# libjxl/libjxl

Measured on AMD Instinct MI355X. Metric: Mpixels/s decode (VarDCT d1.0, 8K RGB), higher is better.
Workload: dtype f32

## Files before the change

libjxl_amd/csrc/kernels_blocks.hip:

```cpp
#include <stdlib.h>
#include <string.h>

#include <type_traits>

#include <initializer_list>

#include "blocks_common.h"
#include "env_switches.h"

namespace jxlhip {

struct StrategyWord {
  uint32_t v[JXLHIP_NUM_STRATEGIES];
};
__host__ __device__ constexpr StrategyWord MakeStrategyWords() {
  StrategyWord w{};
  for (int s = 0; s < JXLHIP_NUM_STRATEGIES; s++)
    w.v[s] = (uint32_t)kCoveredX[s] | ((uint32_t)kCoveredY[s] << 8) | ((uint32_t)(uint8_t)ClassOfStrategy(s) << 16);
  return w;
}
__constant__ StrategyWord kStrategyWords = MakeStrategyWords();

__global__ __launch_bounds__(1024) void k_prepare(DevFrame f, WorkLists wl, uint32_t gy_lo,
                                                  int with_sigma, float epf_quant_mul,
// ... 254 lines not shown
      for (int iy = 0; iy < 4; iy++)
#pragma unroll
        for (int ix = 0; ix < 8; ix++)
          if (ix | iy) block[iy * 8 + ix] = co[(y + iy * 2) * 8 + ix];
      Idct2dReg<4, 8>(block, out);
#pragma unroll
      for (int iy = 0; iy < 4; iy++)
#pragma unroll
        for (int ix = 0; ix < 8; ix++) px[(y * 4 + iy) * 8 + ix] = out[iy * 8 + ix];
    }
  } else if constexpr (STRATEGY == 13) {
    const float b0 = co[0], b1 = co[8];
    const float dcs[2] = {b0 + b1, b0 - b1};
#pragma unroll
    for (int x = 0; x < 2; x++) {
      float block[32], out[32];
      block[0] = dcs[x];
#pragma unroll
      for (int iy = 0; iy < 4; iy++)
#pragma unroll
        for (int ix = 0; ix < 8; ix++)
          if (ix | iy) block[iy * 8 + ix] = co[(x + iy * 2) * 8 + ix];
      Idct2dReg<8, 4>(block, out);
#pragma unroll
      for (int iy = 0; iy < 8; iy++)
#pragma unroll
        for (int ix = 0; ix < 4; ix++) px[iy * 8 + x * 4 + ix] = out[iy * 4 + ix];
    }
  } else {
    AfvToPixels<STRATEGY - 14>(co, px);
  }
}

struct TabOffsets {
  uint32_t v[27];
};
__host__ __device__ constexpr TabOffsets MakeTabOffsets() {
  TabOffsets t{};
  for (int s = 0; s < 27; s++) t.v[s] = DequantOffset(s);
  return t;
}
static constexpr TabOffsets kSingleTabOffset = MakeTabOffsets();

template <typename CT>
struct Dct8Geom {
  static constexpr int kSteps = sizeof(CT) == 2 ? 4 : 2;
  static constexpr uint32_t kPerWg = 4 * kSteps * 8;
};

template <typename CT>
__device__ __forceinline__ void Dct8Rows(const DevFrame& f, const WorkItem* __restrict__ list, uint32_t n,
                                         uint32_t wg) {
  constexpr int kSteps = Dct8Geom<CT>::kSteps;
  const int lane = threadIdx.x & 63, wave = threadIdx.x >> 6;
  const uint32_t first = (wg * 4 + wave) * (kSteps * 8);
  if (first >= n) return;
  const int j = lane >> 3;
  const bool bit3 = (lane & 8) != 0;
  float tab[3][8];
#pragma unroll
  for (int c = 0; c < 3; c++) {
    const float4 t0 = *(const float4*)(f.dequant + c * 64 + j * 8);
    const float4 t1 = *(const float4*)(f.dequant + c * 64 + j * 8 + 4);
    tab[c][0] = t0.x, tab[c][1] = t0.y, tab[c][2] = t0.z, tab[c][3] = t0.w;
    tab[c][4] = t1.x, tab[c][5] = t1.y, tab[c][6] = t1.z, tab[c][7] = t1.w;
  }
  WorkItem it[kSteps];
  Dct8Row<CT> rows[kSteps][3];
  float dcv[kSteps][3];
  bool valid[kSteps];
#pragma unroll
  for (int s = 0; s < kSteps; s++) {
    const uint32_t b = first + s * 8 + (lane & 7);
    valid[s] = b < n;
    it[s] = list[valid[s] ? b : n - 1];
  }
#pragma unroll
  for (int s = 0; s < kSteps; s++) {
    const size_t elem = (size_t)it[s].off * 64u + (size_t)j * 8u;
    const size_t cell = (size_t)(it[s].pos >> 16) * f.xsb + (it[s].pos & 0xffffu);
#pragma unroll
    for (int c = 0; c < 3; c++) {
      rows[s][c].Load(f.coeffs[c], elem);
      dcv[s][c] = f.dc[c][cell];
    }
  }
#pragma unroll
  for (int s = 0; s < kSteps; s++) {
    const BlockHdr h = MakeHdr(f, it[s]);
    int32_t q[8];
    float vy[8];
    rows[s][1].Unpack(q);
#pragma unroll
    for (int k = 0; k < 8; k++) vy[k] = AdjustQuantBias(q[k], f.biases[1], f.biases[3]) * (tab[1][k] * h.sy);
#pragma unroll
    for (int ci = 0; ci < 3; ci++) {
      const int c = ci == 0 ? 1 : (ci == 1 ? 0 : 2);
      float v[8];
      if (c == 1) {
#pragma unroll
        for (int k = 0; k < 8; k++) v[k] = vy[k];
      } else {
        const float sc = c == 0 ? h.sx : h.sb;
        const float cc = c == 0 ? h.x_cc : h.b_cc;
        rows[s][c].Unpack(q);
#pragma unroll
        for (int k = 0; k < 8; k++) {
          const float d = AdjustQuantBias(q[k], f.biases[c], f.biases[3]) * (tab[c][k] * sc);
          v[k] = __builtin_fmaf(cc, vy[k], d);
        }
      }
      if (j == 0) v[0] = dcv[s][c];
      IdctReg<8>(v);
      Transpose8Lanes(v, bit3);
      IdctReg<8>(v);
      if (valid[s]) {
        float* dst = TilePtr(f, c, it[s].pos >> 16, it[s].pos & 0xffffu) + j * 8;
        *(float4*)dst = make_float4(v[0], v[1], v[2], v[3]);
        *(float4*)(dst + 4) = make_float4(v[4], v[5], v[6], v[7]);
      }
    }
  }
}

template <typename CT>
__device__ __forceinline__ void SpecialTask(const DevFrame& f, int strategy, const WorkItem* __restrict__ list,
                                            uint32_t first, uint32_t n, int c) {
  constexpr int kVec = 64 * (int)sizeof(CT) / 16;
  const int lane = threadIdx.x & 63;
  const uint32_t idx = first + lane;
  const bool valid = idx < n;
  const WorkItem it = list[valid ? idx : n - 1];
  const BlockHdr h = MakeHdr(f, it);
  const float* __restrict__ tab = f.dequant + kSingleTabOffset.v[strategy];
  const float dcv = f.dc[c][(size_t)h.aby * f.xsb + h.abx];
  auto unpack = [&](const uint4 r, int32_t* q) {
    const uint32_t w[4] = {r.x, r.y, r.z, r.w};
    if constexpr (sizeof(CT) == 2) {
#pragma unroll
      for (int k = 0; k < 4; k++) {
        q[2 * k] = (int32_t)(int16_t)(w[k] & 0xffffu);
        q[2 * k + 1] = (int32_t)w[k] >> 16;
      }
    } else {
#pragma unroll
      for (int k = 0; k < 4; k++) q[k] = (int32_t)w[k];
    }
  };
  constexpr int kPer = 16 / (int)sizeof(CT);
  float v[64], px[64];
  {
    const uint4* p = (const uint4*)((const CT*)f.coeffs[1] + h.coef);
    uint4 raw[kVec];
#pragma unroll
    for (int i = 0; i < kVec; i++) raw[i] = p[i];
#pragma unroll
    for (int i = 0; i < kVec; i++) {
      int32_t q[kPer];
      unpack(raw[i], q);
#pragma unroll
      for (int k = 0; k < kPer; k++)
        v[i * kPer + k] = AdjustQuantBias(q[k], f.biases[1], f.biases[3]) * (tab[64 + i * kPer + k] * h.sy);
    }
  }
  if (c != 1) {
    const float sc = c == 0 ? h.sx : h.sb;
    const float cc = c == 0 ? h.x_cc : h.b_cc;
    const float bias = c == 0 ? f.biases[0] : f.biases[2];
    const float* __restrict__ tc = tab + c * 64;
    const uint4* p = (const uint4*)((const CT*)f.coeffs[c] + h.coef);
    uint4 raw[kVec];
#pragma unroll
    for (int i = 0; i < kVec; i++) raw[i] = p[i];
#pragma unroll
    for (int i = 0; i < kVec; i++) {
      int32_t q[kPer];
      unpack(raw[i], q);
#pragma unroll
      for (int k = 0; k < kPer; k++) {
        const float d = AdjustQuantBias(q[k], bias, f.biases[3]) * (tc[i * kPer + k] * sc);
        v[i * kPer + k] = __builtin_fmaf(cc, v[i * kPer + k], d);
      }
    }
  }
  v[0] = dcv;
  switch (strategy) {
    case 1: Transform64<1>(v, px); break;
    case 2: Transform64<2>(v, px); break;
    case 3: Transform64<3>(v, px); break;
    case 12: Transform64<12>(v, px); break;
    case 13: Transform64<13>(v, px); break;
    case 14: Transform64<14>(v, px); break;
    case 15: Transform64<15>(v, px); break;
    case 16: Transform64<16>(v, px); break;
    default: Transform64<17>(v, px); break;
  }
  if (valid) {
    float4* dst = (float4*)TilePtr(f, c, h.aby, h.abx);
#pragma unroll
    for (int i = 0; i < 16; i++) dst[i] = make_float4(px[4 * i], px[4 * i + 1], px[4 * i + 2], px[4 * i + 3]);
  }
}

template <typename CT>
__device__ __forceinline__ uint32_t SpecialWorkgroup(const DevFrame& f, const WorkLists& wl, uint32_t wg) {
  uint32_t cnt[kNumSpecial];
  uint32_t tasks = 0;
#pragma unroll
  for (int i = 0; i < kNumSpecial; i++) {
    cnt[i] = wl.count[(kClsSpecial0 + i) * kCounterPad];
    tasks += 3 * ((cnt[i] + 63) / 64);
  }
  const uint32_t special_wgs = (tasks + 3) / 4;
  if (wg >= special_wgs) return special_wgs;
  const uint32_t task = wg * 4 + (threadIdx.x >> 6);
  if (task >= tasks) return special_wgs;
  uint32_t base = 0;
  int cls = -1;
  uint32_t first = 0, n = 0, chan = 0;
#pragma unroll
  for (int i = 0; i < kNumSpecial; i++) {
    const uint32_t t = 3 * ((cnt[i] + 63) / 64);
    if (cls < 0 && task < base + t) {
      cls = i;
      first = ((task - base) / 3) * 64;
      chan = (task - base) % 3;
      n = cnt[i];
    }
    base += t;
  }
  SpecialTask<CT>(f, (int)kSpecialStrategy[cls], wl.list[kClsSpecial0 + cls], first, n,
                  chan == 0 ? 1 : (chan == 1 ? 0 : 2));
  return special_wgs;
}

template <typename CT>
__global__ __launch_bounds__(256, 3) void k_transform_8(DevFrame f, WorkLists wl) {
  const uint32_t special_wgs = SpecialWorkgroup<CT>(f, wl, blockIdx.x);
  if (blockIdx.x >= special_wgs)
    Dct8Rows<CT>(f, wl.list[kClsDct8], wl.count[kClsDct8 * kCounterPad], blockIdx.x - special_wgs);
}

template <int BIT>
__device__ __forceinline__ void ExchangePair(float& a, float& b, int lane) {
  if constexpr (BIT == 5) {
    SwapHalves32(a, b);
  } else if constexpr (BIT == 4) {
    SwapRows16(a, b);
  } else {
    const bool set = (lane >> BIT) & 1;
    const float send = set ? a : b;
    float recv;
    if constexpr (BIT == 3) {
      recv = __int_as_float(__builtin_amdgcn_update_dpp(0, __float_as_int(send), 0x128, 0xf, 0xf, false));
    } else if constexpr (BIT == 2) {
      const float lo = __int_as_float(__builtin_amdgcn_update_dpp(0, __float_as_int(send), 0x124, 0xf, 0xf, false));
      const float hi = __int_as_float(__builtin_amdgcn_update_dpp(0, __float_as_int(send), 0x12c, 0xf, 0xf, false));
      recv = set ? lo : hi;
    } else {
      static_assert(BIT == 1, "lane bits 1..5");
      recv = __int_as_float(__builtin_amdgcn_update_dpp(0, __float_as_int(send), 0x4e, 0xf, 0xf, false));
    }
    a = set ? recv : a;
    b = set ? b : recv;
  }
}

template <int S>
__device__ __forceinline__ void TransposeTile(float* w, int lane) {
  constexpr int kLog = S == 8 ? 3 : (S == 16 ? 4 : 5);
  constexpr int kLb0 = 6 - kLog;
#pragma unroll
  for (int t = kLog - 1; t >= 0; t--) {
#pragma unroll
    for (int k = 0; k < S; k++) {
      if (k & (1 << t)) continue;
      if (kLb0 + t == 5) ExchangePair<5>(w[k], w[k | (1 << t)], lane);
      else if (kLb0 + t == 4) ExchangePair<4>(w[k], w[k | (1 << t)], lane);
      else if (kLb0 + t == 3) ExchangePair<3>(w[k], w[k | (1 << t)], lane);
      else if (kLb0 + t == 2) ExchangePair<2>(w[k], w[k | (1 << t)], lane);
      else ExchangePair<1>(w[k], w[k | (1 << t)], lane);
    }
  }
}

typedef __attribute__((address_space(3))) float LdsTile;
template <int S>
__device__ __forceinline__ void TransposeTileLds(float* w, int b, int j, LdsTile* wave_lds) {
  LdsTile* tile = wave_lds + b * (S * (S + 1));
  LdsTile* row = tile + j * (S + 1);
#pragma unroll
  for (int a = 0; a < S; a++) row[a] = w[a];
  __builtin_amdgcn_fence(__ATOMIC_RELEASE, "wavefront");
  __builtin_amdgcn_wave_barrier();
  __builtin_amdgcn_fence(__ATOMIC_ACQUIRE, "wavefront");
#pragma unroll
  for (int a = 0; a < S; a++) w[a] = tile[a * (S + 1) + j];
  __builtin_amdgcn_fence(__ATOMIC_RELEASE, "wavefront");
  __builtin_amdgcn_wave_barrier();
}
template <int S>
constexpr int TransposeLdsBytes() { return 4 * (64 / S) * S * (S + 1) * 4; }

template <int R, int C, int STRATEGY, typename CT, bool LDS_T = false>
__device__ __forceinline__ void RowLaneUnit(const DevFrame& f, const WorkItem* __restrict__ list,
                                            uint32_t first, uint32_t n, unsigned char* smem = nullptr) {
  constexpr int S = R < C ? R : C, L = R < C ? C : R;
  constexpr int BPS = 64 / S;
  constexpr int CY = R / 8, CX = C / 8;
  constexpr int kTiles = L / S;
  constexpr int kVec = L * (int)sizeof(CT) / 16;
  const int tid = Tid();
  const int lane = tid & 63, wave = tid >> 6;
  const int j = lane / BPS;
  const uint32_t vb = first + wave * BPS + (lane & (BPS - 1));
  if (first + wave * BPS >= n) return;
  const bool valid = vb < n;
  const WorkItem it = list[valid ? vb : n - 1];
  const BlockHdr h = MakeHdr(f, it);
  uint4 raw_a[kVec], raw_b[kVec];
  auto request = [&](int c, uint4* r) {
    const uint4* p = (const uint4*)((const CT*)f.coeffs[c] + h.coef + (size_t)j * L);
#pragma unroll
    for (int i = 0; i < kVec; i++) r[i] = p[i];
  };
  request(1, raw_a);
  request(0, raw_b);
  constexpr int kLlfLanes = CY < CX ? CY : CX;
  constexpr int kLlfRegs = CY < CX ? CX : CY;
  auto llf_of = [&](int c, float* out) {
    const float* dc = f.dc[c] + (size_t)h.aby * f.xsb + h.abx;
    float dp[CY][CX];
#pragma unroll
    for (int x = 0; x < CX; x++) {
      float v[CY];
#pragma unroll
      for (int y = 0; y < CY; y++) v[y] = dc[(size_t)y * f.xsb + x];
      DctReg<CY>(v);
#pragma unroll
      for (int y = 0; y < CY; y++) dp[y][x] = (1.0f / CY) * v[y];
    }
#pragma unroll
    for (int y = 0; y < CY; y++) {
      float v[CX];
#pragma unroll
      for (int x = 0; x < CX; x++) v[x] = dp[y][x];
      DctReg<CX>(v);
      const float ry = kResampleUpHost[CY + y];
#pragma unroll
      for (int x = 0; x < CX; x++) {
        const float val = (1.0f / CX) * v[x];
        if constexpr (CY < CX) {
          if (j == y) out[x] = val * ry * kResampleUpHost[CX + x];
        } else {
          if (j == x) out[y] = val * kResampleUpHost[CX + x] * ry;
        }
      }
    }
  };
  const float* __restrict__ tab = f.dequant + DequantOffset(STRATEGY) + j * L;
  constexpr int kPer = 16 / (int)sizeof(CT);
  auto unpack_piece = [&](const uint4 r, int32_t* q) {
    if constexpr (sizeof(CT) == 2) {
      const uint32_t w[4] = {r.x, r.y, r.z, r.w};
#pragma unroll
      for (int k = 0; k < 4; k++) {
        q[2 * k] = (int32_t)(int16_t)(w[k] & 0xffffu);
        q[2 * k + 1] = (int32_t)w[k] >> 16;
      }
    } else {
      q[0] = (int32_t)r.x, q[1] = (int32_t)r.y, q[2] = (int32_t)r.z, q[3] = (int32_t)r.w;
    }
  };
  float vy[L];
#pragma unroll
  for (int i = 0; i < kVec; i++) {
    int32_t q[kPer];
    unpack_piece(raw_a[i], q);
#pragma unroll
    for (int k = 0; k < kPer; k++)
      vy[i * kPer + k] = AdjustQuantBias(q[k], f.biases[1], f.biases[3]) * (tab[R * C + i * kPer + k] * h.sy);
    if constexpr (L > 16) __builtin_amdgcn_sched_barrier(0);
  }
  request(2, raw_a);
#pragma unroll
  for (int ci = 0; ci < 3; ci++) {
    const int c = ci == 0 ? 1 : (ci == 1 ? 0 : 2);
    float v[L];
    if (c == 1) {
#pragma unroll
      for (int k = 0; k < L; k++) v[k] = vy[k];
    } else {
      const float sc = c == 0 ? h.sx : h.sb;
      const float cc = c == 0 ? h.x_cc : h.b_cc;
#pragma unroll
      for (int i = 0; i < kVec; i++) {
        int32_t q[kPer];
        unpack_piece(c == 0 ? raw_b[i] : raw_a[i], q);
#pragma unroll
        for (int k = 0; k < kPer; k++) {
          const float d = AdjustQuantBias(q[k], f.biases[c], f.biases[3]) * (tab[c * R * C + i * kPer + k] * sc);
          v[i * kPer + k] = __builtin_fmaf(cc, vy[i * kPer + k], d);
        }
        if constexpr (L > 16) __builtin_amdgcn_sched_barrier(0);
      }
    }
    if (j < kLlfLanes) {
      float llf[kLlfRegs];
      llf_of(c, llf);
#pragma unroll
      for (int k = 0; k < kLlfRegs; k++) v[k] = llf[k];
    }
    IdctReg<L>(v);
#pragma unroll
    for (int t = 0; t < kTiles; t++) {
      if constexpr (LDS_T) TransposeTileLds<S>(v + t * S, lane & (BPS - 1), j, (LdsTile*)smem + wave * (BPS * S * (S + 1)));
      else TransposeTile<S>(v + t * S, lane);
    }
#pragma unroll
    for (int t = 0; t < kTiles; t++) IdctReg<S>(v + t * S);
    if constexpr (R < C) {
#pragma unroll
      for (int t = 0; t < kTiles; t++) {
        if constexpr (LDS_T) TransposeTileLds<S>(v + t * S, lane & (BPS - 1), j, (LdsTile*)smem + wave * (BPS * S * (S + 1)));
        else TransposeTile<S>(v + t * S, lane);
      }
      if (valid) {
#pragma unroll
        for (int g = 0; g < C / 8; g++) {
          float* dst = TilePtr(f, c, h.aby + (j >> 3), h.abx + g) + (j & 7) * 8;
          *(float4*)dst = make_float4(v[g * 8], v[g * 8 + 1], v[g * 8 + 2], v[g * 8 + 3]);
          *(float4*)(dst + 4) = make_float4(v[g * 8 + 4], v[g * 8 + 5], v[g * 8 + 6], v[g * 8 + 7]);
        }
      }
    } else {
      if (valid) {
#pragma unroll
        for (int t = 0; t < kTiles; t++) {
          const int a = t * S + j;
#pragma unroll
          for (int g = 0; g < C / 8; g++) {
            float* dst = TilePtr(f, c, h.aby + (a >> 3), h.abx + g) + (a & 7) * 8;
            const float* src = v + t * S + g * 8;
            *(float4*)dst = make_float4(src[0], src[1], src[2], src[3]);
            *(float4*)(dst + 4) = make_float4(src[4], src[5], src[6], src[7]);
          }
        }
      }
    }
  }
}

template <int N>
__device__ __forceinline__ float ResampleUpSel(int i) {
  float r = kResampleUpHost[N];
#pragma unroll
  for (int j = 1; j < N; j++) r = (i == j) ? kResampleUpHost[N + j] : r;
  return r;
}

template <int R, int C>
struct MediumGeom {
  static constexpr int S = R < C ? R : C, L = R < C ? C : R;
  static constexpr int ML = L;
  static constexpr int NB = 64 / ML;
  static constexpr int LP = L + 1;
  static constexpr int TP = C + 1;
  static constexpr int BUF = (S * LP > R * TP ? S * LP : R * TP);
  static constexpr int CY = R / 8, CX = C / 8;
  static constexpr int kUnitVarblocks = (64 / (CY * CX)) > NB ? 64 / (CY * CX) : NB;
  static constexpr int kHdrOffset = (12 * NB * (BUF + CY * CX) + 15) & ~15;
  static constexpr bool kPipelined = (NB * R * C + 767) / 768 <= 2;
  static constexpr int kTabOffset = kHdrOffset + kUnitVarblocks * 48;
  static constexpr int kLdsBytes = kTabOffset + (kPipelined ? 12 * R * C : 0);
};

template <int R, int C, typename CT>
struct MediumLoads {
  using G = MediumGeom<R, C>;
  static constexpr int SIZE = R * C;
  static constexpr int kSteps = (G::NB * SIZE + 767) / 768;
  static constexpr bool kPipelined = G::kPipelined;
  using Raw = typename std::conditional<sizeof(CT) == 2, uint2, int4>::type;
  Raw x[kSteps], y[kSteps], b[kSteps];
  float dc[G::CY];
};

template <typename CT>
__device__ __forceinline__ void UnpackCoeffs(const uint2 v, int32_t* q) {
  q[0] = (int16_t)(v.x & 0xffff);
  q[1] = (int32_t)v.x >> 16;
  q[2] = (int16_t)(v.y & 0xffff);
  q[3] = (int32_t)v.y >> 16;
}
template <typename CT>
__device__ __forceinline__ void UnpackCoeffs(const int4 v, int32_t* q) {
  q[0] = v.x;
  q[1] = v.y;
  q[2] = v.z;
  q[3] = v.w;
}

template <int R, int C, typename CT>
__device__ __forceinline__ void MediumFetch(const DevFrame& f, const BlockHdr* hdr, int nb,
                                            MediumLoads<R, C, CT>& ld) {
  using G = MediumGeom<R, C>;
  using LD = MediumLoads<R, C, CT>;
  using Raw = typename LD::Raw;
  const int tid = Tid();
  const int c = tid >> 6, lane = tid & 63;
  const int b = lane / G::ML, i = lane % G::ML;
  if (b < nb && i < G::CX) {
    const BlockHdr& h = hdr[b];
    const float* dc = f.dc[c] + (size_t)h.aby * f.xsb + h.abx + i;
#pragma unroll
    for (int y = 0; y < G::CY; y++) ld.dc[y] = dc[(size_t)y * f.xsb];
  }
#pragma unroll
  for (int it = 0; it < LD::kSteps; it++) {
    const int k4 = tid * 4 + it * 768;
    if (k4 < nb * LD::SIZE) {
      const int vb = k4 / LD::SIZE, k = k4 % LD::SIZE;
      const size_t at = hdr[vb].coef + k;
      ld.x[it] = *(const Raw*)((const CT*)f.coeffs[0] + at);
      ld.y[it] = *(const Raw*)((const CT*)f.coeffs[1] + at);
      ld.b[it] = *(const Raw*)((const CT*)f.coeffs[2] + at);
    }
  }
}

struct TabStep {
  float4 x, y, b;
};

template <int R, int C, int STRATEGY, typename CT>
__device__ __forceinline__ void MediumBatch(const DevFrame& f, const BlockHdr* hdr, int nb,
                                            const MediumLoads<R, C, CT>& ld, unsigned char* smem) {
  using G = MediumGeom<R, C>;
  using LD = MediumLoads<R, C, CT>;
  constexpr int L = G::L, ML = G::ML, NB = G::NB, LP = G::LP, TP = G::TP, BUF = G::BUF;
  constexpr int CY = G::CY, CX = G::CX;
  constexpr int SIZE = R * C;
  constexpr uint32_t kTab = DequantOffset(STRATEGY);
  float(*buf)[NB][BUF] = reinterpret_cast<float(*)[NB][BUF]>(smem);
  float(*dcp)[NB][CY * CX] = reinterpret_cast<float(*)[NB][CY * CX]>(smem + 12 * NB * BUF);
  const int tid = Tid();

  const int c = tid >> 6, lane = tid & 63;
  const int b = lane / ML, i = lane % ML;
  const bool active = b < nb;
  const int bb = active ? b : 0;
  float* m = &buf[c][bb][0];
  float* dp = &dcp[c][bb][0];

  if (active && i < CX) {
    float v[CY];
    if constexpr (LD::kPipelined) {
#pragma unroll
      for (int y = 0; y < CY; y++) v[y] = ld.dc[y];
    } else {
      const BlockHdr& h = hdr[b];
      const float* dc = f.dc[c] + (size_t)h.aby * f.xsb + h.abx + i;
#pragma unroll
      for (int y = 0; y < CY; y++) v[y] = dc[(size_t)y * f.xsb];
    }
    DctReg<CY>(v);
#pragma unroll
    for (int y = 0; y < CY; y++) dp[y * CX + i] = (1.0f / CY) * v[y];
  }

  const float* __restrict__ tab = f.dequant + kTab;
  auto dequant_step = [&](int k4, const typename LD::Raw rx, const typename LD::Raw ry,
                          const typename LD::Raw rb, const TabStep& t) {
    const int vb = k4 / SIZE, k = k4 % SIZE;
    const BlockHdr& h = hdr[vb];
    int32_t qx[4], qy[4], qb[4];
    UnpackCoeffs<CT>(rx, qx);
    UnpackCoeffs<CT>(ry, qy);
    UnpackCoeffs<CT>(rb, qb);
    const float mx[4] = {t.x.x, t.x.y, t.x.z, t.x.w};
    const float my[4] = {t.y.x, t.y.y, t.y.z, t.y.w};
    const float mb[4] = {t.b.x, t.b.y, t.b.z, t.b.w};
    const int row = k / L, col = k % L;
    float* ox = &buf[0][vb][row * LP + col];
    float* oy = &buf[1][vb][row * LP + col];
    float* ob = &buf[2][vb][row * LP + col];
#pragma unroll
    for (int j = 0; j < 4; j++) {
      const float dy = AdjustQuantBias(qy[j], f.biases[1], f.biases[3]) * (my[j] * h.sy);
      const float dx = AdjustQuantBias(qx[j], f.biases[0], f.biases[3]) * (mx[j] * h.sx);
      const float db = AdjustQuantBias(qb[j], f.biases[2], f.biases[3]) * (mb[j] * h.sb);
      ox[j] = __builtin_fmaf(h.x_cc, dy, dx);
      oy[j] = dy;
      ob[j] = __builtin_fmaf(h.b_cc, dy, db);
    }
  };
  if constexpr (LD::kPipelined) {
    const float* lt = reinterpret_cast<const float*>(smem + G::kTabOffset);
#pragma unroll
    for (int it = 0; it < LD::kSteps; it++) {
      const int k4 = tid * 4 + it * 768;
      if (k4 < nb * SIZE) {
        const int k = k4 % SIZE;
        TabStep t;
        t.x = *(const float4*)(lt + k);
        t.y = *(const float4*)(lt + SIZE + k);
        t.b = *(const float4*)(lt + 2 * SIZE + k);
        dequant_step(k4, ld.x[it], ld.y[it], ld.b[it], t);
      }
    }
  } else {
    using Raw = typename LD::Raw;
    constexpr int kIter = (NB * SIZE + 767) / 768;
    Raw rx[kIter], ry[kIter], rb[kIter];
    TabStep t[kIter];
#pragma unroll
    for (int it = 0; it < kIter; it++) {
      const int k4 = tid * 4 + it * 768;
      if (k4 < nb * SIZE) {
        const int vb = k4 / SIZE, k = k4 % SIZE;
        const size_t at = hdr[vb].coef + k;
        rx[it] = *(const Raw*)((const CT*)f.coeffs[0] + at);
        ry[it] = *(const Raw*)((const CT*)f.coeffs[1] + at);
        rb[it] = *(const Raw*)((const CT*)f.coeffs[2] + at);
        t[it].x = *(const float4*)(tab + k);
        t[it].y = *(const float4*)(tab + SIZE + k);
        t[it].b = *(const float4*)(tab + 2 * SIZE + k);
      }
    }
#pragma unroll
    for (int it = 0; it < kIter; it++) {
      const int k4 = tid * 4 + it * 768;
      if (k4 < nb * SIZE) dequant_step(k4, rx[it], ry[it], rb[it], t[it]);
    }
  }
  __syncthreads();
  if (active && i < CY) {
    float v[CX];
#pragma unroll
    for (int x = 0; x < CX; x++) v[x] = dp[i * CX + x];
    DctReg<CX>(v);
    const float ry = ResampleUpSel<CY>(i);
#pragma unroll
    for (int x = 0; x < CX; x++) {
      const float val = (1.0f / CX) * v[x];
      if constexpr (CY < CX) {
        m[i * LP + x] = val * ry * kResampleUpHost[CX + x];
      } else {
        m[x * LP + i] = val * kResampleUpHost[CX + x] * ry;
      }
    }
  }
  __syncthreads();
  {
    float v[C];
    if (active && i < R) {
#pragma unroll
      for (int j = 0; j < C; j++) v[j] = (R < C) ? m[i * LP + j] : m[j * LP + i];
      IdctReg<C>(v);
    }
    __syncthreads();
    if (active && i < R) {
#pragma unroll
      for (int j = 0; j < C; j++) m[i * TP + j] = v[j];
    }
  }
  __syncthreads();
  if (active && i < C) {
    float v[R];
#pragma unroll
    for (int j = 0; j < R; j++) v[j] = m[j * TP + i];
    IdctReg<R>(v);
#pragma unroll
    for (int j = 0; j < R; j++) m[j * TP + i] = v[j];
  }
  __builtin_amdgcn_wave_barrier();
  {
    constexpr int kParts = SIZE / 4;
    for (int e = lane; e < nb * kParts; e += 64) {
      const int vb = e / kParts, r = e % kParts;
      const int t = r >> 4, part = r & 15;
      const int ty = t / CX, tx = t % CX;
      const float* src = &buf[c][vb][(ty * 8 + (part >> 1)) * TP + tx * 8 + (part & 1) * 4];
      const BlockHdr& h = hdr[vb];
      *(float4*)(TilePtr(f, c, h.aby + ty, h.abx + tx) + part * 4) =
          make_float4(src[0], src[1], src[2], src[3]);
    }
  }
}

template <int R, int C, int STRATEGY, typename CT>
__device__ __forceinline__ void MediumUnit(const DevFrame& f, const WorkItem* __restrict__ list,
                                           uint32_t first, uint32_t n, unsigned char* smem) {
  using G = MediumGeom<R, C>;
  using LD = MediumLoads<R, C, CT>;
  BlockHdr* hdr = reinterpret_cast<BlockHdr*>(smem + G::kHdrOffset);
  const int nvb = (int)min((uint32_t)G::kUnitVarblocks, n - first);
  const int tid0 = Tid();
  if (tid0 < nvb) hdr[tid0] = MakeHdr(f, list[first + tid0]);
  if constexpr (LD::kPipelined) {
    const float4* __restrict__ tab = (const float4*)(f.dequant + DequantOffset(STRATEGY));
    float4* lt = reinterpret_cast<float4*>(smem + G::kTabOffset);
    for (int k = tid0; k < 3 * LD::SIZE / 4; k += 192) lt[k] = tab[k];
  }
  __syncthreads();
  LD cur;
  if constexpr (LD::kPipelined) MediumFetch<R, C, CT>(f, hdr, min(G::NB, nvb), cur);
  for (int b0 = 0; b0 < nvb; b0 += G::NB) {
    LD nxt;
    if constexpr (LD::kPipelined) {
      if (b0 + G::NB < nvb) MediumFetch<R, C, CT>(f, hdr + b0 + G::NB, min(G::NB, nvb - b0 - G::NB), nxt);
    }
    MediumBatch<R, C, STRATEGY, CT>(f, hdr + b0, min(G::NB, nvb - b0), cur, smem);
    __syncthreads();
    if constexpr (LD::kPipelined) cur = nxt;
  }
}

struct APrefetch {
  uint2 x[6], y[6], b[6];
  float dc[8];
};

template <int R, int C, int STRATEGY>
__device__ __forceinline__ void ARequest(const DevFrame& f, const BlockHdr& h, APrefetch& P) {
  using G = MediumGeom<R, C>;
  static_assert(G::NB == 1 && G::ML == 64, "one 64-point varblock per task");
  constexpr int SIZE = R * C;
  constexpr int kIter = (SIZE + 767) / 768;
  static_assert(kIter <= 6 && G::CY <= 8, "APrefetch capacity");
  const int tid = Tid();
  const int c = tid >> 6, lane = tid & 63;
  {
    const float* dc = f.dc[c] + (size_t)h.aby * f.xsb + h.abx + (lane < G::CX ? lane : 0);
#pragma unroll
    for (int y = 0; y < 8; y++) P.dc[y] = y < G::CY ? dc[(size_t)y * f.xsb] : 0.0f;
  }
#pragma unroll
  for (int it = 0; it < 6; it++) {
// ... 145 lines not shown
    for (int i = 0; i < h; i++) tmp[h + i] = v[2 * i + 1];
    IdctMemT<h>(tmp, tmp + N, wc);
#pragma unroll 1
    for (int i = h - 1; i > 0; i--) tmp[h + i] = tmp[h + i] + tmp[h + i - 1];
    tmp[h] = tmp[h] * kSqrt2;
    IdctMemT<h>(tmp + h, tmp + N, wc);
#pragma unroll 1
    for (int i = 0; i < h; i++) {
      const float mul = wc[N + i];
      const float e = tmp[i], o = tmp[h + i];
      v[i] = __builtin_fmaf(mul, o, e);
      v[N - 1 - i] = __builtin_fmaf(-mul, o, e);
    }
  }
}

template <int N>
__device__ __noinline__ void DctMemT(float* v, float* tmp, const float* __restrict__ wc) {
  if constexpr (N == 1) {
    return;
  } else if constexpr (N == 2) {
    const float a = v[0], b = v[1];
    v[0] = a + b;
    v[1] = a - b;
  } else {
    constexpr int h = N / 2;
#pragma unroll 1
    for (int i = 0; i < h; i++) tmp[i] = v[i] + v[N - 1 - i];
    DctMemT<h>(tmp, tmp + N, wc);
#pragma unroll 1
    for (int i = 0; i < h; i++) tmp[h + i] = v[i] - v[N - 1 - i];
#pragma unroll 1
    for (int i = 0; i < h; i++) tmp[h + i] = tmp[h + i] * wc[N + i];
    DctMemT<h>(tmp + h, tmp + N, wc);
    tmp[h] = __builtin_fmaf(tmp[h], kSqrt2, tmp[h + 1]);
#pragma unroll 1
    for (int i = 1; i + 1 < h; i++) tmp[h + i] = tmp[h + i] + tmp[h + i + 1];
#pragma unroll 1
    for (int i = 0; i < h; i++) {
      v[2 * i] = tmp[i];
      v[2 * i + 1] = tmp[h + i];
    }
  }
}

__device__ __forceinline__ void IdctMem(int n, float* v, float* tmp, const float* wc) {
  switch (n) {
    case 32: IdctMemT<32>(v, tmp, wc); break;
    case 64: IdctMemT<64>(v, tmp, wc); break;
    case 128: IdctMemT<128>(v, tmp, wc); break;
    case 256: IdctMemT<256>(v, tmp, wc); break;
    default: break;
  }
}
__device__ __forceinline__ void DctMem(int n, float* v, float* tmp, const float* wc) {
  switch (n) {
    case 2: DctMemT<2>(v, tmp, wc); break;
    case 4: DctMemT<4>(v, tmp, wc); break;
    case 8: DctMemT<8>(v, tmp, wc); break;
    case 16: DctMemT<16>(v, tmp, wc); break;
    case 32: DctMemT<32>(v, tmp, wc); break;
    default: break;
  }
}

template <typename CT>
__global__ __launch_bounds__(256) void k_large(DevFrame f, const WorkItem* __restrict__ list,
                                               const uint32_t* __restrict__ count,
                                               const float* __restrict__ wc,
                                               const float* __restrict__ resample) {
  __shared__ float llf[32 * 33];
  __shared__ float dcs[32 * 33];
  const uint32_t n = *count;
  for (uint32_t item = blockIdx.x; item < n; item += gridDim.x) {
  const BlockHdr h = MakeHdr(f, list[item]);
  const int strategy = f.acs[(size_t)h.aby * f.xsb + h.abx] >> 1;
  const int cx = kCoveredX[strategy], cy = kCoveredY[strategy];
  const int R = cy * 8, C = cx * 8;
  const int L = R < C ? C : R;
  const size_t size = (size_t)R * C;
  const float* __restrict__ tab = f.dequant + DequantOffset(strategy);
  const int tid = threadIdx.x;
  float v[256], tmp[512];
  for (int c = 0; c < 3; c++) {
    for (int i = tid; i < cy * cx; i += 256) {
      const int y = i / cx, x = i % cx;
      dcs[y * 33 + x] = f.dc[c][(size_t)(h.aby + y) * f.xsb + h.abx + x];
    }
    __syncthreads();
    if (tid < cx) {
      for (int y = 0; y < cy; y++) v[y] = dcs[y * 33 + tid];
      DctMem(cy, v, tmp, wc);
      const float sc = 1.0f / cy;
      for (int y = 0; y < cy; y++) dcs[y * 33 + tid] = sc * v[y];
    }
    __syncthreads();
    if (tid < cy) {
      for (int x = 0; x < cx; x++) v[x] = dcs[tid * 33 + x];
      DctMem(cx, v, tmp, wc);
      const float sc = 1.0f / cx;
      for (int x = 0; x < cx; x++) {
        const float val = sc * v[x];
        if (cy < cx) llf[tid * 33 + x] = val * resample[cy + tid] * resample[cx + x];
        else llf[x * 33 + tid] = val * resample[cx + x] * resample[cy + tid];
      }
    }
    __syncthreads();
    const float bias_c = f.biases[c], bias3 = f.biases[3];
    const float sc = c == 0 ? h.sx : (c == 1 ? h.sy : h.sb);
    const float cc = c == 0 ? h.x_cc : (c == 2 ? h.b_cc : 0.0f);
    const int srows = R < C ? R : C;
    const int llf_r = srows / 8, llf_c = L / 8;
    for (int u = tid; u < R; u += 256) {
      for (int j = 0; j < C; j++) {
        const int row = R < C ? u : j, col = R < C ? j : u;
        float val;
        if (row < llf_r && col < llf_c) {
          val = llf[row * 33 + col];
        } else {
          const size_t k = (size_t)row * L + col;
          const int32_t q = LoadCoeff<CT>(f.coeffs[c], h.coef + k);
          val = AdjustQuantBias(q, bias_c, bias3) * (tab[c * size + k] * sc);
          if (c != 1) {
            const int32_t qy = LoadCoeff<CT>(f.coeffs[1], h.coef + k);
            const float dy = AdjustQuantBias(qy, f.biases[1], bias3) * (tab[size + k] * h.sy);
            val = __builtin_fmaf(cc, dy, val);
          }
        }
        v[j] = val;
      }
      IdctMem(C, v, tmp, wc);
      for (int j = 0; j < C; j++) *PlanePtr(f, c, h.aby * 8 + u, h.abx * 8 + j) = v[j];
    }
    __threadfence_block();
    __syncthreads();
    for (int x = tid; x < C; x += 256) {
      for (int j = 0; j < R; j++) v[j] = *PlanePtr(f, c, h.aby * 8 + j, h.abx * 8 + x);
      IdctMem(R, v, tmp, wc);
      for (int j = 0; j < R; j++) *PlanePtr(f, c, h.aby * 8 + j, h.abx * 8 + x) = v[j];
    }
    __syncthreads();
  }
  }
}

struct FamilyEntry {
  int cls;
  int unit_varblocks;
};

struct UnitPick {
  int index;
  int cls;
  uint32_t first;
  uint32_t n;
};

template <int N>
__device__ __forceinline__ UnitPick PickUnit(const FamilyEntry (&fam)[N], const uint32_t* cnt,
                                             uint32_t u) {
  UnitPick p{-1, 0, 0, 0};
  uint32_t base = 0;
#pragma unroll
  for (int i = 0; i < N; i++) {
    const uint32_t units = (cnt[i] + fam[i].unit_varblocks - 1) / fam[i].unit_varblocks;
    if (p.index < 0 && u < base + units) {
      p.index = i;
      p.cls = fam[i].cls;
      p.first = (u - base) * fam[i].unit_varblocks;
      p.n = cnt[i];
    }
    base += units;
  }
  return p;
}

static constexpr int kLdsFamilyA = MediumGeom<64, 64>::kLdsBytes;
static_assert(TransposeLdsBytes<32>() <= kLdsFamilyA && TransposeLdsBytes<16>() <= kLdsFamilyA && TransposeLdsBytes<8>() <= kLdsFamilyA,
              "the row-per-lane units of k_transform_r transpose through family A's allocation");
static_assert(sizeof(BlockHdr) <= 48, "header slots are 48 bytes");
static_assert(MediumGeom<64, 32>::kLdsBytes <= kLdsFamilyA && MediumGeom<32, 64>::kLdsBytes <= kLdsFamilyA, "");

static constexpr FamilyEntry kFamilyA[3] = {{kClsMedium0 + 8, 1}, {kClsMedium0 + 9, 2}, {kClsMedium0 + 10, 2}};
static constexpr FamilyEntry kFamilyR16[3] = {{kClsMedium0 + 2, 16}, {kClsMedium0 + 0, 32}, {kClsMedium0 + 1, 32}};
static constexpr FamilyEntry kFamilyR32[5] = {{kClsMedium0 + 7, 8},  {kClsMedium0 + 5, 16}, {kClsMedium0 + 6, 16},
                                              {kClsMedium0 + 3, 32}, {kClsMedium0 + 4, 32}};
static_assert(kMediumStrategy[8] == 18 && kMediumStrategy[9] == 19 && kMediumStrategy[10] == 20 &&
              kMediumStrategy[7] == 5 && kMediumStrategy[5] == 10 && kMediumStrategy[6] == 11 &&
              kMediumStrategy[2] == 4 && kMediumStrategy[3] == 8 && kMediumStrategy[4] == 9 &&
              kMediumStrategy[0] == 6 && kMediumStrategy[1] == 7, "class table mismatch");

template <int N, typename Body>
__device__ __forceinline__ void UnitDispatch(const FamilyEntry (&fam)[N], const WorkLists& wl,
                                             Body&& body, uint32_t wg_index, uint32_t num_wgs,
                                             uint32_t skip_mask = 0) {
  uint32_t cnt[N];
#pragma unroll
  for (int i = 0; i < N; i++)
    cnt[i] = (skip_mask >> i) & 1u ? 0u : wl.count[fam[i].cls * kCounterPad];
  for (uint32_t u = wg_index;; u += num_wgs) {
    const UnitPick pick = PickUnit(fam, cnt, u);
    if (pick.index < 0) return;
    body(pick.index, wl.list[pick.cls], pick.first, pick.n);
    __syncthreads();
  }
}

static constexpr FamilyEntry kFamilyA1[3] = {{kClsMedium0 + 8, 1}, {kClsMedium0 + 9, 1}, {kClsMedium0 + 10, 1}};

__device__ __forceinline__ void FamilyALoop16(const DevFrame& f, const WorkLists& wl, unsigned char* smem, uint32_t wg_index,
                                              uint32_t num_wgs) {
  uint32_t cnt[3];
#pragma unroll
  for (int i = 0; i < 3; i++) cnt[i] = wl.count[kFamilyA1[i].cls * kCounterPad];
  uint32_t u = wg_index;
  UnitPick cur = PickUnit(kFamilyA1, cnt, u);
  if (cur.index < 0) return;
  BlockHdr hc = MakeHdr(f, wl.list[cur.cls][cur.first]);
  APrefetch P;
#define JXLHIP_AREQUEST(INDEX, H)                      \
  switch (INDEX) {                                     \
    case 0: ARequest<64, 64, 18>(f, H, P); break;      \
    case 1: ARequest<64, 32, 19>(f, H, P); break;      \
    default: ARequest<32, 64, 20>(f, H, P); break;     \
  }
  JXLHIP_AREQUEST(cur.index, hc)
  for (;;) {
    const UnitPick nxt = PickUnit(kFamilyA1, cnt, u + num_wgs);
    WorkItem in{};
    if (nxt.index >= 0) in = wl.list[nxt.cls][nxt.first];
    switch (cur.index) {
      case 0: AHead<64, 64, 18>(f, hc, P, smem); break;
      case 1: AHead<64, 32, 19>(f, hc, P, smem); break;
      default: AHead<32, 64, 20>(f, hc, P, smem); break;
    }
    BlockHdr hn{};
    if (nxt.index >= 0) {
      hn = MakeHdr(f, in);
      JXLHIP_AREQUEST(nxt.index, hn)
    }
    switch (cur.index) {
      case 0: AStore<64, 64>(f, hc, smem); break;
      case 1: AStore<64, 32>(f, hc, smem); break;
      default: AStore<32, 64>(f, hc, smem); break;
    }
    if (nxt.index < 0) return;
    __syncthreads();
    cur = nxt;
    hc = hn;
    u += num_wgs;
  }
#undef JXLHIP_AREQUEST
}

template <typename CT>
__global__ __launch_bounds__(192, sizeof(CT) == 2 ? 3 : 2) void k_transform_a(DevFrame f, WorkLists wl) {
  __shared__ __attribute__((aligned(16))) unsigned char smem[kLdsFamilyA];
  if constexpr (sizeof(CT) == 2) {
    FamilyALoop16(f, wl, smem, blockIdx.x, gridDim.x);
  } else {
    UnitDispatch(kFamilyA, wl,
                 [&](int index, const WorkItem* __restrict__ list, uint32_t first, uint32_t n) {
                   switch (index) {
                     case 0: MediumUnit<64, 64, 18, CT>(f, list, first, n, smem); break;
                     case 1: MediumUnit<64, 32, 19, CT>(f, list, first, n, smem); break;
                     default: MediumUnit<32, 64, 20, CT>(f, list, first, n, smem); break;
                   }
                 },
                 blockIdx.x, gridDim.x);
  }
}

template <typename CT>
__global__ __launch_bounds__(256) void k_transform_r16(DevFrame f, WorkLists wl) {
  UnitDispatch(kFamilyR16, wl,
               [&](int index, const WorkItem* __restrict__ list, uint32_t first, uint32_t n) {
                 switch (index) {
                   case 0: RowLaneUnit<16, 16, 4, CT>(f, list, first, n); break;
                   case 1: RowLaneUnit<16, 8, 6, CT>(f, list, first, n); break;
                   default: RowLaneUnit<8, 16, 7, CT>(f, list, first, n); break;
                 }
               },
               blockIdx.x, gridDim.x, f.mfma16 != nullptr ? 1u : 0u);
}

template <typename CT>
__global__ __launch_bounds__(256) void k_transform_r32(DevFrame f, WorkLists wl) {
  UnitDispatch(kFamilyR32, wl,
               [&](int index, const WorkItem* __restrict__ list, uint32_t first, uint32_t n) {
                 switch (index) {
                   case 0: RowLaneUnit<32, 32, 5, CT>(f, list, first, n); break;
                   case 1: RowLaneUnit<32, 16, 10, CT>(f, list, first, n); break;
                   case 2: RowLaneUnit<16, 32, 11, CT>(f, list, first, n); break;
                   case 3: RowLaneUnit<32, 8, 8, CT>(f, list, first, n); break;
                   default: RowLaneUnit<8, 32, 9, CT>(f, list, first, n); break;
                 }
               },
               blockIdx.x, gridDim.x, f.mfma32 != nullptr ? 1u : 0u);
}

static constexpr FamilyEntry kFamilyR[8] = {{kClsMedium0 + 7, 8},  {kClsMedium0 + 5, 16}, {kClsMedium0 + 6, 16},
                                            {kClsMedium0 + 3, 32}, {kClsMedium0 + 4, 32}, {kClsMedium0 + 2, 16},
                                            {kClsMedium0 + 0, 32}, {kClsMedium0 + 1, 32}};
template <typename CT>
__global__ __launch_bounds__(256, sizeof(CT) == 2 ? 3 : 2) void k_transform_r(DevFrame f, WorkLists wl, uint32_t big_wgs,
                                                                               uint32_t special_wgs, uint32_t r_wgs,
                                                                               uint32_t dct8_wgs) {
  __shared__ __attribute__((aligned(16))) unsigned char smem[kLdsFamilyA];
  if (blockIdx.x < special_wgs) {
    SpecialWorkgroup<CT>(f, wl, blockIdx.x);
    return;
  }
  const uint32_t np = big_wgs + r_wgs;
  const uint32_t i = blockIdx.x - special_wgs;
  const uint32_t need8 = (wl.count[kClsDct8 * kCounterPad] + Dct8Geom<CT>::kPerWg - 1) / Dct8Geom<CT>::kPerWg;
  const uint32_t d8 = need8 * 4 < dct8_wgs ? need8 : dct8_wgs;
  const uint32_t pairs = np < d8 ? np : d8;
  bool is_dct8;
  uint32_t idx;
  if (i < 2 * pairs) {
    is_dct8 = (i & 1u) != 0;
    idx = i >> 1;
  } else {
    is_dct8 = d8 > np;
    idx = i - pairs;
    if (idx >= (is_dct8 ? d8 : np)) return;
  }
  if (is_dct8) {
    Dct8Rows<CT>(f, wl.list[kClsDct8], wl.count[kClsDct8 * kCounterPad], idx);
    return;
  }
  if (idx < big_wgs) {
    if (threadIdx.x >= 192) return;
    if constexpr (sizeof(CT) == 2) {
      FamilyALoop16(f, wl, smem, idx, big_wgs);
    } else {
      UnitDispatch(kFamilyA, wl,
                   [&](int index, const WorkItem* __restrict__ list, uint32_t first, uint32_t n) {
                     switch (index) {
                       case 0: MediumUnit<64, 64, 18, CT>(f, list, first, n, smem); break;
                       case 1: MediumUnit<64, 32, 19, CT>(f, list, first, n, smem); break;
                       default: MediumUnit<32, 64, 20, CT>(f, list, first, n, smem); break;
                     }
                   },
                   idx, big_wgs);
    }
    return;
  }
  UnitDispatch(kFamilyR, wl,
               [&](int index, const WorkItem* __restrict__ list, uint32_t first, uint32_t n) {
                 switch (index) {
                   case 0: RowLaneUnit<32, 32, 5, CT, true>(f, list, first, n, smem); break;
                   case 1: RowLaneUnit<32, 16, 10, CT, true>(f, list, first, n, smem); break;
                   case 2: RowLaneUnit<16, 32, 11, CT, true>(f, list, first, n, smem); break;
                   case 3: RowLaneUnit<32, 8, 8, CT, true>(f, list, first, n, smem); break;
                   case 4: RowLaneUnit<8, 32, 9, CT, true>(f, list, first, n, smem); break;
                   case 5: RowLaneUnit<16, 16, 4, CT, true>(f, list, first, n, smem); break;
                   case 6: RowLaneUnit<16, 8, 6, CT, true>(f, list, first, n, smem); break;
                   default: RowLaneUnit<8, 16, 7, CT, true>(f, list, first, n, smem); break;
                 }
               },
               idx - big_wgs, r_wgs, (f.mfma32 != nullptr ? 1u : 0u) | (f.mfma16 != nullptr ? 1u << 5 : 0u));
}

template <typename CT>
static void LaunchBlocksT(const DevFrame& f, const WorkLists& wl, uint32_t cells, const float* wc,
                          const float* resample, hipStream_t st, const FilterParams* emit) {
  const uint32_t units = cells / 64;
  const uint32_t grid_l = cells / 128 < 512u ? (cells / 128 ? cells / 128 : 1) : 512u;
  constexpr uint32_t kDct8PerWg = Dct8Geom<CT>::kPerWg;
  uint32_t grid_a = units + 3 < 1536u ? units + 3 : 1536u;
  uint32_t grid_r16 = units + 3 < 4096u ? units + 3 : 4096u;
  uint32_t grid_r32 = units / 2 + 5 < 3072u ? units / 2 + 5 : 3072u;
  const int big_env = jxlhip_env::Get().big_wgs.load(std::memory_order_relaxed);
  const int r_env = jxlhip_env::Get().r_wgs.load(std::memory_order_relaxed);
  const bool big_set = big_env >= 1 && big_env <= 4096;
  if (big_set && (uint32_t)big_env < grid_a) grid_a = (uint32_t)big_env;
  if (r_env >= 1 && r_env <= 4096) {
    if ((uint32_t)r_env < grid_r16) grid_r16 = (uint32_t)r_env;
    if ((uint32_t)r_env < grid_r32) grid_r32 = (uint32_t)r_env;
  }
  auto any = [&](std::initializer_list<int> strategies) {
    if (f.used_acs == 0) return true;
    for (int s : strategies)
      if (f.used_acs & (1u << s)) return true;
    return false;
  };
  const bool need_r16 = any({6, 7}) || (!f.mfma16 && any({4}));
  const bool need_r32 = any({8, 9, 10, 11}) || (!f.mfma32 && any({5}));
  const bool merged_r = need_r16 && need_r32;
  const bool have_big = any({18, 19, 20});
  bool specials_in_r = false, dct8_in_r = false;
  uint32_t grid_specials = 0, grid_dct8 = 0;
  if (have_big && !merged_r)
    hipLaunchKernelGGL((k_transform_a<CT>), dim3(grid_a), dim3(192), 0, st, f, wl);
  {
    const bool specials = any({1, 2, 3, 12, 13, 14, 15, 16, 17});
    const uint32_t bound_s = specials ? (cells / 64 + kNumSpecial) * 3 / 4 + 1 : 0;
    const uint32_t cells_8 = f.fused == 0 ? cells : (f.fused == 2 ? 2u * f.xsb : 0u);
    const uint32_t bound_8 = (any({0}) && cells_8) ? (cells_8 + kDct8PerWg - 1) / kDct8PerWg : 0;
    const uint32_t grid_8 = (bound_s > bound_8 ? bound_s : bound_8) + (specials ? kNumSpecial : 0);
    specials_in_r = merged_r && specials;
    dct8_in_r = merged_r && bound_8 != 0;
    grid_specials = bound_s + kNumSpecial;
    grid_dct8 = bound_8;
    if (grid_8 && !merged_r) hipLaunchKernelGGL((k_transform_8<CT>), dim3(grid_8), dim3(256), 0, st, f, wl);
  }
  if (merged_r) {
    const uint32_t big_cap = big_set ? (uint32_t)big_env : 512u;
    const uint32_t big_wgs = have_big ? (grid_a < big_cap ? grid_a : big_cap) : 0u;
    const uint32_t special_wgs = specials_in_r ? grid_specials : 0u;
    const uint32_t dct8_wgs = dct8_in_r ? grid_dct8 : 0u;
    hipLaunchKernelGGL((k_transform_r<CT>), dim3(special_wgs + big_wgs + grid_r16 + dct8_wgs), dim3(256), 0, st, f, wl,
                       big_wgs, special_wgs, grid_r16, dct8_wgs);
  } else {
    if (need_r16) hipLaunchKernelGGL((k_transform_r16<CT>), dim3(grid_r16), dim3(256), 0, st, f, wl);
    if (need_r32) hipLaunchKernelGGL((k_transform_r32<CT>), dim3(grid_r32), dim3(256), 0, st, f, wl);
  }
  if (f.mfma32 && any({5})) LaunchMfma32(f, wl, cells, st, emit);
  if (f.mfma16 && any({4})) LaunchMfma16(f, wl, cells, st);
  if (cells >= 256 && any({21, 22, 23, 24, 25, 26}))
    hipLaunchKernelGGL(k_large<CT>, dim3(grid_l), dim3(256), 0, st, f, wl.list[kClsLarge],
                       wl.count + kClsLarge * kCounterPad, wc, resample);
}

void LaunchPrepare(const DevFrame& f, const WorkLists& wl, int with_sigma, float epf_quant_mul,
                   const SharpLut& lut, hipStream_t st) {
  uint32_t lo = f.band_g0, hi = f.band_g1;
  if (with_sigma) {
    if (lo > 0) lo--;
    if (hi < f.ysg) hi++;
  }
  hipLaunchKernelGGL(k_prepare, dim3(f.xsg * (hi - lo)), dim3(1024), 0, st, f, wl, lo,
                     with_sigma, epf_quant_mul, lut);
}

void LaunchBlocks(const DevFrame& f, const WorkLists& wl, uint32_t cells, const float* wc,
                  const float* resample, hipStream_t st, const FilterParams* emit) {
  if (f.coeff_type == JXLHIP_COEFF_I16)
    LaunchBlocksT<int16_t>(f, wl, cells, wc, resample, st, emit);
  else
    LaunchBlocksT<int32_t>(f, wl, cells, wc, resample, st, emit);
}

}
```

Baseline: 130,900.

## Stage per-class dequant tables in LDS and prefetch DC for row-lane units

Family-R work now runs through a dedicated loop. The loop copies the active strategy's dequant table into LDS (with padded rows) whenever the class changes, and the row-lane units read their dequant weights from LDS instead of global memory. The DC values used for the LLF are loaded early: all channels up front for short rows, or one channel ahead after each IDCT otherwise, so their latency overlaps compute. Stores are also made unconditional, so padding lanes rewrite duplicate data instead of branching. In exchange there is a block-wide barrier after every unit, table refills on class switches, and more registers held for the prefetched DC values.

Result: slower. 125,000 (-4.5%).

```diff
diff --git a/libjxl_amd/csrc/kernels_blocks.hip b/libjxl_amd/csrc/kernels_blocks.hip
--- a/libjxl_amd/csrc/kernels_blocks.hip
+++ b/libjxl_amd/csrc/kernels_blocks.hip
@@ -580,6 +580,31 @@
 template <int S>
 constexpr int TransposeLdsBytes() { return 4 * (64 / S) * S * (S + 1) * 4; }
 
+static constexpr int kRowLaneTabOffset = TransposeLdsBytes<32>();
+template <int R, int C>
+constexpr int RowLaneTabStride() { return (R < C ? C : R) + 4; }
+template <int R, int C>
+constexpr int RowLaneTabBytes() { return 3 * (R < C ? R : C) * RowLaneTabStride<R, C>() * 4; }
+typedef float __attribute__((ext_vector_type(4))) RawVec4;
+typedef __attribute__((address_space(3))) RawVec4 LdsVec4;
+
+template <int R, int C, int STRATEGY>
+__device__ __forceinline__ void RowLaneTabFill(const DevFrame& f, unsigned char* smem) {
+  constexpr int S = R < C ? R : C, L = R < C ? C : R, LP = RowLaneTabStride<R, C>();
+  const float4* __restrict__ src = (const float4*)(f.dequant + DequantOffset(STRATEGY));
+  LdsTile* dst = (LdsTile*)(smem + kRowLaneTabOffset);
+  const int tid = Tid();
+#pragma unroll
+  for (int k0 = 0; k0 < 3 * S * L / 4; k0 += 256) {
+    const int k = k0 + tid;
+    if (3 * S * L / 4 % 256 == 0 || k < 3 * S * L / 4) {
+      const int row = k / (L / 4), col = k % (L / 4);
+      const float4 q = src[k];
+      *(LdsVec4*)(dst + row * LP + col * 4) = RawVec4{q.x, q.y, q.z, q.w};
+    }
+  }
+}
+
 template <int R, int C, int STRATEGY, typename CT, bool LDS_T = false>
 __device__ __forceinline__ void RowLaneUnit(const DevFrame& f, const WorkItem* __restrict__ list,
                                             uint32_t first, uint32_t n, unsigned char* smem = nullptr) {
@@ -606,14 +631,21 @@
   request(0, raw_b);
   constexpr int kLlfLanes = CY < CX ? CY : CX;
   constexpr int kLlfRegs = CY < CX ? CX : CY;
-  auto llf_of = [&](int c, float* out) {
+  auto dc_request = [&](int c, float* raw) {
     const float* dc = f.dc[c] + (size_t)h.aby * f.xsb + h.abx;
+#pragma unroll
+    for (int y = 0; y < CY; y++) {
+#pragma unroll
+      for (int x = 0; x < CX; x++) raw[y * CX + x] = dc[(size_t)y * f.xsb + x];
+    }
+  };
+  auto llf_from = [&](const float* raw, float* out) {
     float dp[CY][CX];
 #pragma unroll
     for (int x = 0; x < CX; x++) {
       float v[CY];
 #pragma unroll
-      for (int y = 0; y < CY; y++) v[y] = dc[(size_t)y * f.xsb + x];
+      for (int y = 0; y < CY; y++) v[y] = raw[y * CX + x];
       DctReg<CY>(v);
 #pragma unroll
       for (int y = 0; y < CY; y++) dp[y][x] = (1.0f / CY) * v[y];
@@ -636,8 +668,35 @@
       }
     }
   };
+  constexpr bool kDcEarly = LDS_T;
+  constexpr bool kStoreAll = LDS_T;
+  constexpr bool kDcAllAtHead = kDcEarly && L <= 16;
+  float dcr[3][CY * CX];
+  if constexpr (kDcEarly) {
+    if (j < kLlfLanes) {
+      dc_request(1, dcr[1]);
+      if constexpr (kDcAllAtHead) {
+        dc_request(0, dcr[0]);
+        dc_request(2, dcr[2]);
+      }
+    }
+  }
+  constexpr int kPer = 16 / (int)sizeof(CT);
+  constexpr int kTabChan = LDS_T ? S * RowLaneTabStride<R, C>() : R * C;
   const float* __restrict__ tab = f.dequant + DequantOffset(STRATEGY) + j * L;
-  constexpr int kPer = 16 / (int)sizeof(CT);
+  const LdsTile* tab_lds = (const LdsTile*)(smem + kRowLaneTabOffset) + j * RowLaneTabStride<R, C>();
+  auto tab_piece = [&](int c, int i, float* t) {
+    if constexpr (LDS_T) {
+#pragma unroll
+      for (int k = 0; k < kPer; k += 4) {
+        const RawVec4 q = *(const LdsVec4*)(tab_lds + c * kTabChan + i * kPer + k);
+        t[k] = q.x, t[k + 1] = q.y, t[k + 2] = q.z, t[k + 3] = q.w;
+      }
+    } else {
+#pragma unroll
+      for (int k = 0; k < kPer; k++) t[k] = tab[c * kTabChan + i * kPer + k];
+    }
+  };
   auto unpack_piece = [&](const uint4 r, int32_t* q) {
     if constexpr (sizeof(CT) == 2) {
       const uint32_t w[4] = {r.x, r.y, r.z, r.w};
@@ -655,9 +714,11 @@
   for (int i = 0; i < kVec; i++) {
     int32_t q[kPer];
     unpack_piece(raw_a[i], q);
+    float t[kPer];
+    tab_piece(1, i, t);
 #pragma unroll
     for (int k = 0; k < kPer; k++)
-      vy[i * kPer + k] = AdjustQuantBias(q[k], f.biases[1], f.biases[3]) * (tab[R * C + i * kPer + k] * h.sy);
+      vy[i * kPer + k] = AdjustQuantBias(q[k], f.biases[1], f.biases[3]) * (t[k] * h.sy);
     if constexpr (L > 16) __builtin_amdgcn_sched_barrier(0);
   }
   request(2, raw_a);
@@ -675,9 +736,11 @@
       for (int i = 0; i < kVec; i++) {
         int32_t q[kPer];
         unpack_piece(c == 0 ? raw_b[i] : raw_a[i], q);
+        float t[kPer];
+        tab_piece(c, i, t);
 #pragma unroll
         for (int k = 0; k < kPer; k++) {
-          const float d = AdjustQuantBias(q[k], f.biases[c], f.biases[3]) * (tab[c * R * C + i * kPer + k] * sc);
+          const float d = AdjustQuantBias(q[k], f.biases[c], f.biases[3]) * (t[k] * sc);
           v[i * kPer + k] = __builtin_fmaf(cc, vy[i * kPer + k], d);
         }
         if constexpr (L > 16) __builtin_amdgcn_sched_barrier(0);
@@ -685,7 +748,8 @@
     }
     if (j < kLlfLanes) {
       float llf[kLlfRegs];
-      llf_of(c, llf);
+      if constexpr (!kDcEarly) dc_request(c, dcr[c]);
+      llf_from(dcr[c], llf);
 #pragma unroll
       for (int k = 0; k < kLlfRegs; k++) v[k] = llf[k];
     }
@@ -697,13 +761,16 @@
     }
 #pragma unroll
     for (int t = 0; t < kTiles; t++) IdctReg<S>(v + t * S);
+    if constexpr (kDcEarly && !kDcAllAtHead) {
+      if (ci < 2 && j < kLlfLanes) dc_request(ci == 0 ? 0 : 2, dcr[ci == 0 ? 0 : 2]);
+    }
     if constexpr (R < C) {
 #pragma unroll
       for (int t = 0; t < kTiles; t++) {
         if constexpr (LDS_T) TransposeTileLds<S>(v + t * S, lane & (BPS - 1), j, (LdsTile*)smem + wave * (BPS * S * (S + 1)));
         else TransposeTile<S>(v + t * S, lane);
       }
-      if (valid) {
+      if (valid || kStoreAll) {
 #pragma unroll
         for (int g = 0; g < C / 8; g++) {
           float* dst = TilePtr(f, c, h.aby + (j >> 3), h.abx + g) + (j & 7) * 8;
@@ -712,7 +779,7 @@
         }
       }
     } else {
-      if (valid) {
+      if (valid || kStoreAll) {
 #pragma unroll
         for (int t = 0; t < kTiles; t++) {
           const int a = t * S + j;
@@ -1464,6 +1531,52 @@
 static constexpr FamilyEntry kFamilyR[8] = {{kClsMedium0 + 7, 8},  {kClsMedium0 + 5, 16}, {kClsMedium0 + 6, 16},
                                             {kClsMedium0 + 3, 32}, {kClsMedium0 + 4, 32}, {kClsMedium0 + 2, 16},
                                             {kClsMedium0 + 0, 32}, {kClsMedium0 + 1, 32}};
+static_assert(kRowLaneTabOffset % 16 == 0 && kRowLaneTabOffset >= TransposeLdsBytes<16>() && kRowLaneTabOffset >= TransposeLdsBytes<8>() &&
+                  kRowLaneTabOffset + RowLaneTabBytes<32, 32>() <= kLdsFamilyA && kRowLaneTabOffset + RowLaneTabBytes<32, 16>() <= kLdsFamilyA &&
+                  kRowLaneTabOffset + RowLaneTabBytes<16, 32>() <= kLdsFamilyA && kRowLaneTabOffset + RowLaneTabBytes<32, 8>() <= kLdsFamilyA &&
+                  kRowLaneTabOffset + RowLaneTabBytes<8, 32>() <= kLdsFamilyA && kRowLaneTabOffset + RowLaneTabBytes<16, 16>() <= kLdsFamilyA &&
+                  kRowLaneTabOffset + RowLaneTabBytes<16, 8>() <= kLdsFamilyA && kRowLaneTabOffset + RowLaneTabBytes<8, 16>() <= kLdsFamilyA,
+              "transposition tiles + the resident class's dequant table fit family A's allocation, for all eight classes");
+
+template <typename CT>
+__device__ __forceinline__ void FamilyRLoop(const DevFrame& f, const WorkLists& wl, unsigned char* smem, uint32_t wg_index,
+                                            uint32_t num_wgs, uint32_t skip_mask) {
+  uint32_t cnt[8];
+#pragma unroll
+  for (int i = 0; i < 8; i++) cnt[i] = (skip_mask >> i) & 1u ? 0u : wl.count[kFamilyR[i].cls * kCounterPad];
+  int resident = -1;
+  for (uint32_t u = wg_index;; u += num_wgs) {
+    const UnitPick pick = PickUnit(kFamilyR, cnt, u);
+    if (pick.index < 0) return;
+    const WorkItem* __restrict__ list = wl.list[pick.cls];
+    if (pick.index != resident) {
+      switch (pick.index) {
+        case 0: RowLaneTabFill<32, 32, 5>(f, smem); break;
+        case 1: RowLaneTabFill<32, 16, 10>(f, smem); break;
+        case 2: RowLaneTabFill<16, 32, 11>(f, smem); break;
+        case 3: RowLaneTabFill<32, 8, 8>(f, smem); break;
+        case 4: RowLaneTabFill<8, 32, 9>(f, smem); break;
+        case 5: RowLaneTabFill<16, 16, 4>(f, smem); break;
+        case 6: RowLaneTabFill<16, 8, 6>(f, smem); break;
+        default: RowLaneTabFill<8, 16, 7>(f, smem); break;
+      }
+      resident = pick.index;
+      __syncthreads();
+    }
+    switch (pick.index) {
+      case 0: RowLaneUnit<32, 32, 5, CT, true>(f, list, pick.first, pick.n, smem); break;
+      case 1: RowLaneUnit<32, 16, 10, CT, true>(f, list, pick.first, pick.n, smem); break;
+      case 2: RowLaneUnit<16, 32, 11, CT, true>(f, list, pick.first, pick.n, smem); break;
+      case 3: RowLaneUnit<32, 8, 8, CT, true>(f, list, pick.first, pick.n, smem); break;
+      case 4: RowLaneUnit<8, 32, 9, CT, true>(f, list, pick.first, pick.n, smem); break;
+      case 5: RowLaneUnit<16, 16, 4, CT, true>(f, list, pick.first, pick.n, smem); break;
+      case 6: RowLaneUnit<16, 8, 6, CT, true>(f, list, pick.first, pick.n, smem); break;
+      default: RowLaneUnit<8, 16, 7, CT, true>(f, list, pick.first, pick.n, smem); break;
+    }
+    __syncthreads();
+  }
+}
+
 template <typename CT>
 __global__ __launch_bounds__(256, sizeof(CT) == 2 ? 3 : 2) void k_transform_r(DevFrame f, WorkLists wl, uint32_t big_wgs,
                                                                                uint32_t special_wgs, uint32_t r_wgs,
@@ -1509,20 +1622,7 @@
     }
     return;
   }
-  UnitDispatch(kFamilyR, wl,
-               [&](int index, const WorkItem* __restrict__ list, uint32_t first, uint32_t n) {
-                 switch (index) {
-                   case 0: RowLaneUnit<32, 32, 5, CT, true>(f, list, first, n, smem); break;
-                   case 1: RowLaneUnit<32, 16, 10, CT, true>(f, list, first, n, smem); break;
-                   case 2: RowLaneUnit<16, 32, 11, CT, true>(f, list, first, n, smem); break;
-                   case 3: RowLaneUnit<32, 8, 8, CT, true>(f, list, first, n, smem); break;
-                   case 4: RowLaneUnit<8, 32, 9, CT, true>(f, list, first, n, smem); break;
-                   case 5: RowLaneUnit<16, 16, 4, CT, true>(f, list, first, n, smem); break;
-                   case 6: RowLaneUnit<16, 8, 6, CT, true>(f, list, first, n, smem); break;
-                   default: RowLaneUnit<8, 16, 7, CT, true>(f, list, first, n, smem); break;
-                 }
-               },
-               idx - big_wgs, r_wgs, (f.mfma32 != nullptr ? 1u : 0u) | (f.mfma16 != nullptr ? 1u << 5 : 0u));
+  FamilyRLoop<CT>(f, wl, smem, idx - big_wgs, r_wgs, (f.mfma32 != nullptr ? 1u : 0u) | (f.mfma16 != nullptr ? 1u << 5 : 0u));
 }
 
 template <typename CT>
```
